# KaranSankla/Lidar_Object_Detection

Hardware: AMD Instinct MI355X
Metric: LiDAR points/sec projected+instance-labelled (higher is better)
Workload: dtype f64

## Files before the change

### lidar_object_detection_amd/csrc/lpf_kernels.hip.h

```cpp
#pragma once
#include <hip/hip_runtime.h>
#include <stdint.h>

#define LPF_BLOCK 256
#define LPF_SEG_QUANTUM 4096
#define LPF_SEG_SMALL 1024
#define LPF_GROUP_SEGS 64
#define LPF_FRM_SHARDS 8
#define LPF_MAX_MASKS_DEV 32
#define LPF_TAB_ROWS 36
#define LPF_TAB_GROUPS 9

struct LpfFrame {
    long long pt_off;
    long long inst_base;
    int N;
    int seg_off;
    int nseg;
    int box_off;
    int B;
    int pad;
    long long cand_off;
    int cand_words;
    int grp_off;
    int shift;
    int pad4;
};

struct LpfParams {
    double T[12];
    double K[9];
    double dmin, dmax;
    int W, H;
    int F, M;
    int seg_pts;
    int nseg_total;
    int nseg_cap;
    int ngrp_cap;
    int oriented;
    long long inst_cap;
    LpfFrame frame0;
    const LpfFrame *frames;
    const LpfFrame *segs;
    const int2 *blks;
    const int4 *cblks;
    int nblk, ncblk;
    int lists_small;
    int csplit;
    const float4 *pts;
    const void *label_img;
    const int4 *rects;
    const uint32_t *rect_grid;
    int rg_cw, rg_cells;
    const double *boxp;
    const float *boxq;
    const unsigned long long *cand;
    int2 *uv;
    uint32_t *label_bits;
    double *depth, *uf, *vf;
    long long *valid_idx;
    int2 *uv_valid;
    uint32_t *label_valid;
    long long *inst_idx;
    int32_t *count_out;
    void *summary;
    unsigned long long *vbal, *mbal;
    uint4 *seg_tab;
    uint4 *grp_tab;
    uint4 *frm_tab;
    uint4 *seg_pre;
    unsigned *cnt;
    float4 *mlist;
    int count_boxes;
    int count_lazy;
    int tile_pts;
};

__device__ __forceinline__ int lpf_lane() { return threadIdx.x & 63; }
__device__ __forceinline__ int lpf_wave() { return threadIdx.x >> 6; }

__device__ __forceinline__ int lpf_xcd_remap(int b, int n)
{
    const int q = n >> 3, r = n & 7, x = b & 7, i = b >> 3;
    return (x < r ? x * (q + 1) : r * (q + 1) + (x - r) * q) + i;
}

__device__ __forceinline__ int lpf_find_frame(const LpfFrame *frames, int F, int sid)
{
    int lo = 0, hi = F;
    while (hi - lo > 1) {
        const int mid = (lo + hi) >> 1;
        if (frames[mid].seg_off <= sid) lo = mid; else hi = mid;
    }
    return lo;
}

__device__ __forceinline__ int lpf_uni(int v) { return __builtin_amdgcn_readfirstlane(v); }
__device__ __forceinline__ long long lpf_uni64(long long v)
{
    return (long long)(((unsigned long long)(unsigned)lpf_uni((int)((unsigned long long)v >> 32)) << 32) | (unsigned)lpf_uni((int)v));
}
__device__ __forceinline__ LpfFrame lpf_frame_record(const LpfFrame &by_value, const LpfFrame *table, const bool many, const int idx)
{
    LpfFrame fr = by_value;
    if (many) {
        const LpfFrame t = table[lpf_uni(idx)];
        fr.pt_off = lpf_uni64(t.pt_off); fr.inst_base = lpf_uni64(t.inst_base); fr.N = lpf_uni(t.N); fr.seg_off = lpf_uni(t.seg_off);
        fr.nseg = lpf_uni(t.nseg); fr.box_off = lpf_uni(t.box_off); fr.B = lpf_uni(t.B); fr.pad = lpf_uni(t.pad);
        fr.cand_off = lpf_uni64(t.cand_off); fr.cand_words = lpf_uni(t.cand_words); fr.grp_off = lpf_uni(t.grp_off); fr.shift = lpf_uni(t.shift);
    }
    return fr;
}

__device__ __forceinline__ int32_t lpf_sat_i32(double r)
{
    int v;
    asm("v_cvt_i32_f64 %0, %1" : "=v"(v) : "v"(r));
    return (r != r) ? INT32_MIN : v;
}

__device__ __forceinline__ unsigned lpf_expo(double x) { return ((unsigned)__double2hiint(x) >> 20) & 0x7ffu; }

__device__ __forceinline__ void lpf_div2(double qx, double qy, double ad, double &uf, double &vf)
{
    const unsigned ea = lpf_expo(ad), ex = lpf_expo(qx), ey = lpf_expo(qy);
    const unsigned lo = min(ea, min(ex, ey)), hi = max(ea, max(ex, ey));
    if (lo >= 723u && hi <= 1323u) {
        double r = __builtin_amdgcn_rcp(ad);
        double e = fma(-ad, r, 1.0); r = fma(r, e, r);
        e = fma(-ad, r, 1.0);        r = fma(r, e, r);
        double q = qx * r; double s = fma(-ad, q, qx); uf = fma(s, r, q);
        q = qy * r;        s = fma(-ad, q, qy);        vf = fma(s, r, q);
    } else {
        uf = qx / ad;
        vf = qy / ad;
    }
}

__device__ __forceinline__ void lpf_project_point(const LpfParams &P, float fx, float fy, float fz,
                                                  double &uf, double &vf, double &d)
{
    const double x = (double)fx, y = (double)fy, z = (double)fz;
    double cx = P.T[0] * x; cx = fma(P.T[1], y, cx); cx = fma(P.T[2],  z, cx); cx = cx + P.T[3];
    double cy = P.T[4] * x; cy = fma(P.T[5], y, cy); cy = fma(P.T[6],  z, cy); cy = cy + P.T[7];
    double cz = P.T[8] * x; cz = fma(P.T[9], y, cz); cz = fma(P.T[10], z, cz); cz = cz + P.T[11];
    double qx = P.K[0] * cx; qx = fma(P.K[1], cy, qx); qx = fma(P.K[2], cz, qx);
    double qy = P.K[3] * cx; qy = fma(P.K[4], cy, qy); qy = fma(P.K[5], cz, qy);
    d = P.K[6] * cx; d = fma(P.K[7], cy, d); d = fma(P.K[8], cz, d);
    if (d == 0.0) d = -1e-6;
    lpf_div2(qx, qy, fabs(d), uf, vf);
}

__device__ __forceinline__ void lpf_project_point_mem(const double *__restrict__ TK, float fx, float fy, float fz,
                                                      double &uf, double &vf, double &d)
{
    const double x = (double)fx, y = (double)fy, z = (double)fz;
    double cx = TK[0] * x; cx = fma(TK[1], y, cx); cx = fma(TK[2],  z, cx); cx = cx + TK[3];
    double cy = TK[4] * x; cy = fma(TK[5], y, cy); cy = fma(TK[6],  z, cy); cy = cy + TK[7];
    double cz = TK[8] * x; cz = fma(TK[9], y, cz); cz = fma(TK[10], z, cz); cz = cz + TK[11];
    double qx = TK[12] * cx; qx = fma(TK[13], cy, qx); qx = fma(TK[14], cz, qx);
    double qy = TK[15] * cx; qy = fma(TK[16], cy, qy); qy = fma(TK[17], cz, qy);
    d = TK[18] * cx; d = fma(TK[19], cy, d); d = fma(TK[20], cz, d);
    if (d == 0.0) d = -1e-6;
    lpf_div2(qx, qy, fabs(d), uf, vf);
}

__device__ __forceinline__ unsigned lpf_f32_to_u8(float v)
{
    int t;
    if (!(v > -2147483904.0f && v < 2147483648.0f)) t = INT32_MIN; else t = (int)v;
    return (unsigned)t & 0xFFu;
}

template <typename T, int MODE>
__device__ __forceinline__ bool lpf_member(T v)
{
    if (MODE == 0) return v != 0;
    if (MODE == 1) return lpf_f32_to_u8((float)v) != 0u;
    if (MODE == 3) return (float)v > 0.5f;
    return lpf_f32_to_u8((float)v * 255.0f) == 255u;
}

template <typename T, int MODE> struct LpfDirect { };
template <typename LT> struct LpfIsDirect { static constexpr bool value = false; };
template <typename T, int MODE> struct LpfIsDirect<LpfDirect<T, MODE> > { static constexpr bool value = true; };

template <typename T, int MODE> struct LpfDirectRect { };
template <typename LT> struct LpfIsDirectRect { static constexpr bool value = false; };
template <typename T, int MODE> struct LpfIsDirectRect<LpfDirectRect<T, MODE> > { static constexpr bool value = true; };
template <typename T, int MODE> struct LpfIsDirect<LpfDirectRect<T, MODE> > { static constexpr bool value = true; };

template <typename LT>
struct LpfLabelSrc {
    typedef LT elem;
    static __device__ __forceinline__ uint32_t get(const elem *__restrict__ img, const LpfParams &, const int pix, const int4 *, int, int) { return (uint32_t)img[pix]; }
    static __device__ __forceinline__ size_t frame_stride(const LpfParams &P) { return (size_t)P.W * (size_t)P.H; }
};
template <typename T, int MODE>
struct LpfLabelSrc<LpfDirect<T, MODE> > {
    typedef T elem;
    static __device__ __forceinline__ uint32_t get(const elem *__restrict__ msk, const LpfParams &P, const int pix, const int4 *__restrict__ rc,
                                                   const int ui, const int vi)
    {
        const size_t hw = (size_t)P.W * (size_t)P.H;
        uint32_t l = 0;
        for (int m0 = 0; m0 < P.M; m0 += 8) {
            T v[8];
#pragma unroll
            for (int j = 0; j < 8; ++j) v[j] = msk[(size_t)min(m0 + j, P.M - 1) * hw + pix];
#pragma unroll
            for (int j = 0; j < 8; ++j)
                if (m0 + j < P.M && lpf_member<T, MODE>(v[j])) l |= 1u << (m0 + j);
        }
        if (rc && l) {
            uint32_t rest = l;
            while (rest) {
                const int m = __ffs(rest) - 1;
                rest &= rest - 1u;
                const int4 q = rc[m];
                if (!(ui >= q.x && ui < q.z && vi >= q.y && vi < q.w)) l &= ~(1u << m);
            }
        }
        return l;
    }
    static __device__ __forceinline__ size_t frame_stride(const LpfParams &P) { return (size_t)P.M * (size_t)P.W * (size_t)P.H; }
};

template <typename T, int MODE>
struct LpfLabelSrc<LpfDirectRect<T, MODE> > {
    typedef T elem;
    static constexpr int mode = MODE;
    static __device__ __forceinline__ uint32_t get(const elem *__restrict__, const LpfParams &, const int, const int4 *, int, int) { return 0u; }
    static __device__ __forceinline__ size_t frame_stride(const LpfParams &P) { return (size_t)P.M * (size_t)P.W * (size_t)P.H; }
};

#define LPF_F_X4 1u
#define LPF_F_NTLOAD 2u
#define LPF_F_NTSTORE 4u
#define LPF_F_LAB_NOMATH 8u
#define LPF_F_LAB_NOGATHER 16u
#define LPF_F_LAB_NOSTORE 32u

#define LPF_F_LAB_NOBAL 64u
#define LPF_F_LAB_NOTAB 128u

#define LPF_RG_SHIFT 4
#define LPF_RG_CELL (1 << LPF_RG_SHIFT)
__device__ __forceinline__ unsigned lpf_wave_or(unsigned x);

template <int ROWS, unsigned FL, typename LT, bool PRELOADED>
__device__ __forceinline__ void lpf_k1_tile(const LpfParams &P, const int blk, unsigned *s_cnt, float4 (&p)[ROWS])
{
    constexpr int TILE = LPF_BLOCK * ROWS;
    static_assert(LPF_SEG_QUANTUM % TILE == 0 && (LPF_SEG_SMALL % TILE == 0 || ROWS >= 8), "tiles must divide segments (8-row and larger tiles: large geometry only)");
    const int tid = threadIdx.x, lane = lpf_lane(), wave = lpf_wave();
    const int tiles_per_seg = P.seg_pts / TILE;
    const int lb = lpf_xcd_remap(blk, P.nseg_total * tiles_per_seg);
    const int sid = lb / tiles_per_seg;
    LpfFrame fr = P.frame0;
    if (P.F > 1) fr = P.segs[__builtin_amdgcn_readfirstlane(sid)];
    const int f = fr.pad;
    const int sh = fr.shift;
    const long long pbase = fr.pt_off - sh;
    const int seg_start = (sid - fr.seg_off) * P.seg_pts;
    const int seg_end = min(seg_start + P.seg_pts, fr.N + sh);
    const int c = seg_start + (lb - sid * tiles_per_seg) * TILE;
    if (c >= seg_end) return;
    const float4 *__restrict__ pts = P.pts + pbase;
    typedef LpfLabelSrc<LT> Src;
    const typename Src::elem *__restrict__ limg =
        (P.label_img && P.M > 0) ? static_cast<const typename Src::elem *>(P.label_img) + (size_t)f * Src::frame_stride(P) : nullptr;
    const int rows_per_seg = P.seg_pts >> 6;
    if (tid < LPF_TAB_ROWS) s_cnt[tid] = 0;
    __syncthreads();
    unsigned nvalid_w = 0, nmask_w = 0;

    {
        const int wbase = c + wave * (ROWS * 64) + lane;
#pragma unroll
        for (int r = 0; r < ROWS; ++r) {
            if constexpr (PRELOADED) continue;
            const float4 *src = pts + min(wbase + r * 64, seg_end - 1);
            if (FL & LPF_F_NTLOAD) {
                typedef float f4v __attribute__((ext_vector_type(4)));
                const f4v t = __builtin_nontemporal_load(reinterpret_cast<const f4v *>(src));
                p[r] = make_float4(t.x, t.y, t.z, t.w);
            } else {
                p[r] = *src;
            }
        }
        uint32_t lab[ROWS];
        bool valid[ROWS];
        constexpr bool RECT = LpfIsDirectRect<LT>::value;
        const int4 *__restrict__ rc_f = ((RECT || LpfIsDirect<LT>::value) && P.rects) ? P.rects + (size_t)f * P.M : nullptr;
        const uint32_t *__restrict__ rgrid = (RECT && limg && P.rect_grid) ? P.rect_grid + (size_t)f * P.rg_cells : nullptr;
        const size_t mhw = (size_t)P.W * (size_t)P.H;
        unsigned long long myv = 0, mym = 0;
        auto consume = [&](const int r, uint32_t l, const bool okr) {
            const int idx = wbase + r * 64;
            if (idx >= sh && idx < seg_end && P.label_bits && !(FL & LPF_F_LAB_NOSTORE)) {
                if (FL & LPF_F_NTSTORE) __builtin_nontemporal_store(l, P.label_bits + pbase + idx);
                else P.label_bits[pbase + idx] = l;
            }
            const unsigned long long vb = __ballot(okr);
            const unsigned long long mb = __ballot(l != 0);
            if (lane == r) { myv = vb; mym = mb; }
            if (l && P.mlist && !(FL & LPF_F_LAB_NOSTORE))
                P.mlist[pbase + (wbase - lane) + ((wbase - lane) == 0 ? sh : 0) + nmask_w + __popcll(mb & ((1ull << lane) - 1ull))] =
                    make_float4(p[r].x, p[r].y, p[r].z, __uint_as_float(l));
            nvalid_w += __popcll(vb);
            nmask_w += __popcll(mb);
            while (l) {
                const int m = __ffs(l) - 1;
                l &= l - 1;
                atomicAdd(&s_cnt[2 + m], 1u);
            }
        };
#pragma unroll
        for (int r = 0; r < ROWS; ++r) {
            const int idx = wbase + r * 64;
            const bool live = idx >= sh && idx < seg_end;
            if (FL & LPF_F_X4) asm volatile("" ::"v"(p[r].w));
            double uf, vf, d, ru, rv;
            if (FL & LPF_F_LAB_NOMATH) {
                uf = (double)p[r].x; vf = (double)p[r].y; d = (double)p[r].z;
                ru = uf + 700.0; rv = vf + 100.0;
            } else {
                lpf_project_point(P, p[r].x, p[r].y, p[r].z, uf, vf, d);
                ru = rint(uf); rv = rint(vf);
            }
            const int ui = lpf_sat_i32(ru), vi = lpf_sat_i32(rv);
            const bool ok = live && ((unsigned)ui < (unsigned)P.W) && ((unsigned)vi < (unsigned)P.H) &&
                            (d > P.dmin) && (d < P.dmax);
            valid[r] = ok;
            lab[r] = 0;
            if constexpr (RECT) {
                if (ok && rgrid) lab[r] = rgrid[(vi >> LPF_RG_SHIFT) * P.rg_cw + (ui >> LPF_RG_SHIFT)];
            } else
            if (!(FL & LPF_F_LAB_NOGATHER)) {
                if (ok && limg) lab[r] = Src::get(limg, P, vi * P.W + ui, rc_f, ui, vi);
            }
            if (live && !(FL & LPF_F_LAB_NOSTORE)) {
                const long long g = pbase + idx;
                if (P.uv) {
                    if (FL & LPF_F_NTSTORE) {
                        typedef int i2v __attribute__((ext_vector_type(2)));
                        i2v t; t.x = ui; t.y = vi;
                        __builtin_nontemporal_store(t, reinterpret_cast<i2v *>(P.uv + g));
                    } else {
                        P.uv[g] = make_int2(ui, vi);
                    }
                }
                if (P.depth) P.depth[g] = d;
                if (P.uf) P.uf[g] = uf;
                if (P.vf) P.vf[g] = vf;
            }
        }
#pragma unroll
        for (int r = 0; r < ROWS; ++r) {
            uint32_t l = lab[r];
            if constexpr (RECT) {
                if (__any(l != 0u)) {
                    double uf, vf, d;
                    lpf_project_point(P, p[r].x, p[r].y, p[r].z, uf, vf, d);
                    const int ui = lpf_sat_i32(rint(uf)), vi = lpf_sat_i32(rint(vf));
                    const unsigned pix = (unsigned)(vi * P.W + ui);
                    uint32_t any = lpf_wave_or(l), l2 = 0u;
                    while (any) {
                        const int m = __ffs(any) - 1;
                        any &= any - 1u;
                        const int4 q = rc_f[m];
                        const bool in = ((l >> m) & 1u) && ui >= q.x && ui < q.z && vi >= q.y && vi < q.w;
                        if (__any(in)) {
                            const typename Src::elem *__restrict__ mk = limg + (size_t)m * mhw;
                            if (in && lpf_member<typename Src::elem, Src::mode>(mk[pix])) l2 |= 1u << m;
                        }
                    }
                    l = l2;
                }
            }
            consume(r, l, valid[r]);
        }
        if (lane < ROWS && !(FL & LPF_F_LAB_NOBAL)) {
            const size_t row = (size_t)sid * rows_per_seg + ((c - seg_start) >> 6) + wave * ROWS + lane;
            P.vbal[row] = myv;
            P.mbal[row] = mym;
        }
    }
    if (lane == 0) { atomicAdd(&s_cnt[0], nvalid_w); atomicAdd(&s_cnt[1], nmask_w); }
    __syncthreads();
    if (!(FL & LPF_F_LAB_NOTAB)) {
        if (tid < (2 + P.M + 1) >> 1) {
            const unsigned long long v = (unsigned long long)s_cnt[2 * tid] | ((unsigned long long)s_cnt[2 * tid + 1] << 32);
            if (v) {
                int seg_off = P.frame0.seg_off, grp_off = P.frame0.grp_off, fid = P.frame0.pad;
                if (P.F > 1) { const LpfFrame *e = P.segs + lpf_uni(sid); seg_off = e->seg_off; grp_off = e->grp_off; fid = e->pad; }
                const int k = sid - seg_off, g = tid >> 1, h = tid & 1;
                atomicAdd(reinterpret_cast<unsigned long long *>(P.seg_tab + (size_t)g * P.nseg_cap + sid) + h, v);
                atomicAdd(reinterpret_cast<unsigned long long *>(P.grp_tab + (size_t)g * P.ngrp_cap + grp_off + (k >> 6)) + h, v);
                atomicAdd(reinterpret_cast<unsigned long long *>(P.frm_tab + ((size_t)fid * LPF_FRM_SHARDS + (k & (LPF_FRM_SHARDS - 1))) * LPF_TAB_GROUPS + g) + h, v);
            }
        }
    }
}

template <int ROWS, unsigned FL, typename LT>
__device__ __forceinline__ void lpf_k1_tile(const LpfParams &P, const int blk, unsigned *s_cnt)
{
    float4 p[ROWS];
    lpf_k1_tile<ROWS, FL, LT, false>(P, blk, s_cnt, p);
}

template <int ROWS, unsigned FL, typename LT = uint32_t>
__global__ __launch_bounds__(LPF_BLOCK) void lpf_k1_project_t(const LpfParams P)
{
    __shared__ unsigned s_cnt[LPF_TAB_ROWS];
    lpf_k1_tile<ROWS, FL, LT>(P, (int)blockIdx.x, s_cnt);
}

#define LPF_K1_FLAGS (LPF_F_X4 | LPF_F_NTLOAD | LPF_F_NTSTORE)

__device__ __forceinline__ bool lpf_oriented_inside(double px, double py, double pz, const double *__restrict__ b)
{
    const double rx = px - b[0], ry = py - b[1], rz = pz - b[2];
    const bool exact_ok = b[15] != 0.0;
#pragma unroll
    for (int a = 0; a < 3; ++a) {
        const double v0 = b[3 + 4 * a], v1 = b[4 + 4 * a], v2 = b[5 + 4 * a], vv = b[6 + 4 * a];
        double d = v1 * ry; d = fma(v0, rx, d); d = fma(v2, rz, d);
        bool in;
        if (exact_ok && !(fabs(d) < 1e-200 && d != 0.0)) {
            in = (d >= 0.0) && (d <= vv);
        } else {
            const double t = d / vv;
            in = (t >= 0.0) && (t <= 1.0);
        }
        if (!in) return false;
    }
    return true;
}

__device__ __forceinline__ bool lpf_aabb_inside(double px, double py, double pz, const double *__restrict__ b)
{
    return (px >= b[0]) && (px <= b[3]) && (py >= b[1]) && (py <= b[4]) && (pz >= b[2]) && (pz <= b[5]);
}

__device__ __forceinline__ unsigned lpf_rl(unsigned v, int l) { return (unsigned)__builtin_amdgcn_readlane((int)v, l); }
__device__ __forceinline__ float lpf_rlf(float v, int l) { return __int_as_float(__builtin_amdgcn_readlane(__float_as_int(v), l)); }
__device__ __forceinline__ unsigned long long lpf_rl64(unsigned long long v, int l)
{
    return (unsigned long long)lpf_rl((unsigned)v, l) | ((unsigned long long)lpf_rl((unsigned)(v >> 32), l) << 32);
}
#define LPF_DPP_ADD(x, ctrl, rows) ((x) + (unsigned)__builtin_amdgcn_update_dpp(0, (int)(x), (ctrl), (rows), 0xf, false))
__device__ __forceinline__ unsigned lpf_wave_sum(unsigned x)
{
    x = LPF_DPP_ADD(x, 0xB1, 0xf);
    x = LPF_DPP_ADD(x, 0x4E, 0xf);
    x = LPF_DPP_ADD(x, 0x141, 0xf);
    x = LPF_DPP_ADD(x, 0x140, 0xf);
    x = LPF_DPP_ADD(x, 0x142, 0xa);
    x = LPF_DPP_ADD(x, 0x143, 0xc);
    return lpf_rl(x, 63);
}
__device__ __forceinline__ unsigned lpf_sum8(unsigned x)
{
    x = LPF_DPP_ADD(x, 0xB1, 0xf);
    x = LPF_DPP_ADD(x, 0x4E, 0xf);
    x = LPF_DPP_ADD(x, 0x141, 0xf);
    return lpf_rl(x, 0);
}
__device__ __forceinline__ unsigned lpf_wave_or(unsigned x)
{
#define LPF_DPP_OR(x, ctrl, rows) ((x) | (unsigned)__builtin_amdgcn_update_dpp(0, (int)(x), (ctrl), (rows), 0xf, false))
    x = LPF_DPP_OR(x, 0xB1, 0xf); x = LPF_DPP_OR(x, 0x4E, 0xf); x = LPF_DPP_OR(x, 0x141, 0xf); x = LPF_DPP_OR(x, 0x140, 0xf);
    x = LPF_DPP_OR(x, 0x142, 0xa); x = LPF_DPP_OR(x, 0x143, 0xc);
#undef LPF_DPP_OR
    return lpf_rl(x, 63);
}

__device__ __forceinline__ void lpf_block_excl4(const unsigned sum[4], unsigned excl[4], unsigned all[4],
                                                unsigned (*s_wsum)[4], int lane, int wave)
{
    unsigned inc[4];
#pragma unroll
    for (int j = 0; j < 4; ++j) {
        unsigned x = sum[j];
#pragma unroll
        for (int o = 1; o < 64; o <<= 1) {
            const unsigned t = __shfl_up(x, o);
            if (lane >= o) x += t;
        }
        inc[j] = x;
        if (lane == 63) s_wsum[wave][j] = x;
    }
    __syncthreads();
#pragma unroll
    for (int j = 0; j < 4; ++j) {
        unsigned wo = 0, a = 0;
#pragma unroll
        for (int w = 0; w < 4; ++w) { const unsigned t = s_wsum[w][j]; if (w < wave) wo += t; a += t; }
        excl[j] = wo + inc[j] - sum[j];
        all[j] = a;
    }
    __syncthreads();
}

__global__ __launch_bounds__(LPF_BLOCK) void lpf_scan_segments(const LpfParams P)
{
    __shared__ unsigned s_toff[LPF_TAB_GROUPS][LPF_BLOCK][4];
    __shared__ unsigned s_wsum[4][4], s_tot[LPF_TAB_ROWS], s_off[LPF_TAB_ROWS];
    const int f = blockIdx.x, tid = threadIdx.x, lane = lpf_lane(), wave = lpf_wave();
    const LpfFrame fr = lpf_frame_record(P.frame0, P.frames, P.F > 1, f);
    const int seg_lo = fr.seg_off, seg_hi = fr.seg_off + fr.nseg;
    const int ngroups = (2 + P.M + 3) >> 2;
    const int R = (fr.nseg + LPF_BLOCK - 1) / LPF_BLOCK;
    const int my_lo = min(seg_lo + tid * R, seg_hi), my_hi = min(my_lo + R, seg_hi);
    for (int g = 0; g < ngroups; ++g) {
        const uint4 *__restrict__ row = P.seg_tab + (size_t)g * P.nseg_cap;
        unsigned sum[4] = {0, 0, 0, 0};
#pragma unroll 8
        for (int sg = my_lo; sg < my_hi; ++sg) {
            const uint4 v = row[sg];
            sum[0] += v.x; sum[1] += v.y; sum[2] += v.z; sum[3] += v.w;
        }
        unsigned excl[4], all[4];
        lpf_block_excl4(sum, excl, all, s_wsum, lane, wave);
#pragma unroll
        for (int j = 0; j < 4; ++j) { s_toff[g][tid][j] = excl[j]; if (tid == 0) s_tot[4 * g + j] = all[j]; }
    }
    __syncthreads();
    if (tid < LPF_TAB_ROWS) {
        const bool used = tid < 4 * ngroups;
        unsigned off = 0;
        if (used) for (int c = 2; c < tid; ++c) off += s_tot[c];
        s_off[tid] = off;
    }
    __syncthreads();
    for (int g = 0; g < ngroups; ++g) {
        const uint4 *__restrict__ row = P.seg_tab + (size_t)g * P.nseg_cap;
        uint4 *__restrict__ pre = P.seg_pre + (size_t)g * P.nseg_cap;
        unsigned run[4];
#pragma unroll
        for (int j = 0; j < 4; ++j) run[j] = s_off[4 * g + j] + s_toff[g][tid][j];
#pragma unroll 8
        for (int sg = my_lo; sg < my_hi; ++sg) {
            const uint4 v = row[sg];
            pre[sg] = make_uint4(run[0], run[1], run[2], run[3]);
            run[0] += v.x; run[1] += v.y; run[2] += v.z; run[3] += v.w;
        }
    }
}

#define LPF_LISTS_WAVES 4
#define LPF_LIST_CAP 1024


__device__ __forceinline__ void lpf_bits_to_list(unsigned long long rowbits, unsigned rowbase, int lane, unsigned short *lst)
{
    unsigned pos = rowbase;
    const unsigned short tag = (unsigned short)(lane * 64);
    while (rowbits) {
        const int b = __ffsll((long long)rowbits) - 1;
        rowbits &= rowbits - 1ull;
        lst[pos++] = (unsigned short)(tag + b);
    }
}

template <bool PRE, int STEP>
__device__ __forceinline__ void lpf_list_prefix(const LpfParams &P, const LpfFrame &fr, const int sid, unsigned &bef, unsigned &tot)
{
    const int lane = lpf_lane();
    const int ngroups = (2 + P.M + 3) >> 2;
    const int k = sid - fr.seg_off;
    bef = 0; tot = 0;
    if (PRE) {
        uint4 q = make_uint4(0u, 0u, 0u, 0u);
        if (lane < ngroups) q = P.seg_pre[(size_t)lane * P.nseg_cap + sid];
        const int g = min(lane >> 2, LPF_TAB_GROUPS - 1);
        const unsigned x = __shfl(q.x, g), y = __shfl(q.y, g), z = __shfl(q.z, g), w = __shfl(q.w, g);
        bef = ((lane & 3) == 0) ? x : ((lane & 3) == 1) ? y : ((lane & 3) == 2) ? z : w;
    } else {
        const int gi = k >> 6, j = k & 63;
        for (int g0 = 0; g0 < ngroups; g0 += STEP) {
            uint4 a[STEP], b[STEP], t[STEP];
#pragma unroll
            for (int u = 0; u < STEP; ++u) {
                const int g = g0 + u;
                a[u] = make_uint4(0u, 0u, 0u, 0u); b[u] = a[u]; t[u] = a[u];
                if (g < ngroups) {
                    if (lane < j) a[u] = P.seg_tab[(size_t)g * P.nseg_cap + fr.seg_off + (gi << 6) + lane];
                    if (lane < gi) b[u] = P.grp_tab[(size_t)g * P.ngrp_cap + fr.grp_off + lane];
                    if (lane < LPF_FRM_SHARDS) t[u] = P.frm_tab[((size_t)fr.pad * LPF_FRM_SHARDS + lane) * LPF_TAB_GROUPS + g];
                }
            }
#pragma unroll
            for (int u = 0; u < STEP; ++u) {
                const int g = g0 + u;
                if (g >= ngroups) break;
                const unsigned px = lpf_wave_sum(a[u].x + b[u].x), py = lpf_wave_sum(a[u].y + b[u].y), pz = lpf_wave_sum(a[u].z + b[u].z), pw = lpf_wave_sum(a[u].w + b[u].w);
                const unsigned tx = lpf_sum8(t[u].x), ty = lpf_sum8(t[u].y), tz = lpf_sum8(t[u].z), tw = lpf_sum8(t[u].w);
                if ((lane >> 2) == g) {
                    bef = ((lane & 3) == 0) ? px : ((lane & 3) == 1) ? py : ((lane & 3) == 2) ? pz : pw;
                    tot = ((lane & 3) == 0) ? tx : ((lane & 3) == 1) ? ty : ((lane & 3) == 2) ? tz : tw;
                }
            }
        }
    }
}

template <bool PRE>
__device__ __forceinline__ unsigned lpf_list_posreg(const LpfParams &P, const unsigned bef, const unsigned tot)
{
    const int lane = lpf_lane();
    if (PRE) return (unsigned)__shfl((int)bef, (lane + 2) & 63);
    unsigned off = (lane >= 2 && lane < 2 + P.M) ? tot : 0u;
    const unsigned own = off;
#pragma unroll
    for (int o = 1; o < 64; o <<= 1) {
        const unsigned u = __shfl_up(off, o);
        if (lane >= o) off += u;
    }
    return (unsigned)__shfl((int)(off - own + bef), (lane + 2) & 63);
}

template <bool PRE, int STEP>
__device__ __forceinline__ void lpf_lists_wave(const LpfParams &P, const LpfFrame &fr, const int sid, unsigned short *lst)
{
    const int lane = lpf_lane();
    const unsigned long long lt = (1ull << lane) - 1ull;
    const int rps = P.seg_pts >> 6;
    const int k = sid - fr.seg_off;
    unsigned long long vb = 0, mb = 0;
    if (lane < rps) {
        vb = P.vbal[(size_t)sid * rps + lane];
        mb = P.mbal[(size_t)sid * rps + lane];
    }
    unsigned bef, tot;
    lpf_list_prefix<PRE, STEP>(P, fr, sid, bef, tot);
    const int sh = fr.shift;
    const int seg_start = k * P.seg_pts;
    const int seg_end = min(seg_start + P.seg_pts, fr.N + sh);
    const int nrows = (seg_end - seg_start + 63) >> 6;
    if (lane >= nrows) { vb = 0; mb = 0; }
    const unsigned cv = __popcll(vb), cm = __popcll(mb);
    unsigned iv = cv, im = cm;
#pragma unroll
    for (int o = 1; o < 64; o <<= 1) {
        const unsigned tv = __shfl_up(iv, o), tm = __shfl_up(im, o);
        if (lane >= o) { iv += tv; im += tm; }
    }
    const unsigned vbase = iv - cv, mbase = im - cm;
    const unsigned nv = lpf_rl(iv, 63), L = lpf_rl(im, 63);
    const long long run_v = (long long)lpf_rl(bef, 0);

    if (P.valid_idx && nv) {
        long long *__restrict__ dst = P.valid_idx + fr.pt_off + run_v;
        const long long o = fr.pt_off + run_v, g0 = fr.pt_off - sh + seg_start;
        const long long room = (long long)fr.N - run_v;
        if (nv > (unsigned)LPF_LIST_CAP || nv > 6u * (unsigned)nrows) {
            for (int r = 0; r < nrows; ++r) {
                const unsigned long long rv = lpf_rl64(vb, r);
                if (rv == 0ull) continue;
                const long long pos = lpf_rl(vbase, r) + __popcll(rv & lt);
                if (((rv >> lane) & 1ull) && pos < room) {
                    dst[pos] = (long long)(seg_start + r * 64 + lane - sh);
                    if (P.uv_valid) P.uv_valid[o + pos] = P.uv[g0 + r * 64 + lane];
                    if (P.label_valid) P.label_valid[o + pos] = P.label_bits[g0 + r * 64 + lane];
                }
            }
        } else {
            lpf_bits_to_list(vb, vbase, lane, lst);
            __builtin_amdgcn_wave_barrier();
            for (unsigned e = lane; e < nv && (long long)e < room; e += 64) {
                const int pt = seg_start + (int)lst[e] - sh;
                dst[e] = (long long)pt;
                if (P.uv_valid) P.uv_valid[o + e] = P.uv[fr.pt_off + pt];
                if (P.label_valid) P.label_valid[o + e] = P.label_bits[fr.pt_off + pt];
            }
            __builtin_amdgcn_wave_barrier();
        }
    }
    if (L == 0 || P.inst_idx == nullptr) return;

    unsigned posreg = lpf_list_posreg<PRE>(P, bef, tot);
    const float4 *__restrict__ mseg = P.mlist + (fr.pt_off - sh) + seg_start;
    const int rows_per_wave = P.tile_pts >> 8;
    const int rpw_shift = (rows_per_wave == 8) ? 3 : (rows_per_wave == 4) ? 2 : (rows_per_wave == 2) ? 1 : 0;
    const int dead0 = (seg_start == 0) ? sh : 0;

    for (int r0 = 0; r0 < nrows;) {
// ... 1360 lines not shown
```

Measured before the change: 171.8 billion.

## Add fast path for full tiles and batch rect-mask refinement gathers

Adds a specialised FAST path for tiles that lie entirely inside the segment and use only the common outputs (uv plus labels, no depth or float coordinates). That path drops the bounds clamps and per-row liveness checks, turns label gathers into unconditional loads, and ballots validity during projection. For the rect-grid label type it keeps the projected pixel coordinates in registers instead of re-projecting in the refinement loop, and reads rectangles through the scalar constant address space. It also processes mask candidates four at a time so their gathers are issued together. The cost is more code instantiated per template, more register pressure from the extra per-row arrays, and a path split on a runtime condition.

```diff
diff --git a/lidar_object_detection_amd/csrc/lpf_kernels.hip.h b/lidar_object_detection_amd/csrc/lpf_kernels.hip.h
--- a/lidar_object_detection_amd/csrc/lpf_kernels.hip.h
+++ b/lidar_object_detection_amd/csrc/lpf_kernels.hip.h
@@ -247,6 +247,10 @@
 #define LPF_RG_SHIFT 4
 #define LPF_RG_CELL (1 << LPF_RG_SHIFT)
 __device__ __forceinline__ unsigned lpf_wave_or(unsigned x);
+__device__ __forceinline__ unsigned long long lpf_rl64(unsigned long long v, int l);
+template <bool B> struct LpfBool { static constexpr bool value = B; };
+typedef int lpf_int4v __attribute__((ext_vector_type(4)));
+typedef const __attribute__((address_space(4))) lpf_int4v *LpfConstRects;
 
 template <int ROWS, unsigned FL, typename LT, bool PRELOADED>
 __device__ __forceinline__ void lpf_k1_tile(const LpfParams &P, const int blk, unsigned *s_cnt, float4 (&p)[ROWS])
@@ -275,12 +279,21 @@
     __syncthreads();
     unsigned nvalid_w = 0, nmask_w = 0;
 
-    {
+    constexpr bool RECT = LpfIsDirectRect<LT>::value;
+    const int4 *__restrict__ rc_f = ((RECT || LpfIsDirect<LT>::value) && P.rects) ? P.rects + (size_t)(RECT ? lpf_uni(f) : f) * P.M : nullptr;
+    const uint32_t *__restrict__ rgrid = (RECT && limg && P.rect_grid) ? P.rect_grid + (size_t)f * P.rg_cells : nullptr;
+    auto rows = [&](auto fast_tag) {
+        constexpr bool FAST = decltype(fast_tag)::value;
+        constexpr bool STORE = !(FL & LPF_F_LAB_NOSTORE);
+        int2 *const o_uv = P.uv;
+        uint32_t *const o_lab = P.label_bits;
+        double *const o_depth = FAST ? nullptr : P.depth, *const o_uf = FAST ? nullptr : P.uf, *const o_vf = FAST ? nullptr : P.vf;
+        float4 *const o_mlist = P.mlist;
         const int wbase = c + wave * (ROWS * 64) + lane;
 #pragma unroll
         for (int r = 0; r < ROWS; ++r) {
             if constexpr (PRELOADED) continue;
-            const float4 *src = pts + min(wbase + r * 64, seg_end - 1);
+            const float4 *src = pts + (FAST ? wbase + r * 64 : min(wbase + r * 64, seg_end - 1));
             if (FL & LPF_F_NTLOAD) {
                 typedef float f4v __attribute__((ext_vector_type(4)));
                 const f4v t = __builtin_nontemporal_load(reinterpret_cast<const f4v *>(src));
@@ -290,25 +303,35 @@
             }
         }
         uint32_t lab[ROWS];
-        bool valid[ROWS];
-        constexpr bool RECT = LpfIsDirectRect<LT>::value;
-        const int4 *__restrict__ rc_f = ((RECT || LpfIsDirect<LT>::value) && P.rects) ? P.rects + (size_t)f * P.M : nullptr;
-        const uint32_t *__restrict__ rgrid = (RECT && limg && P.rect_grid) ? P.rect_grid + (size_t)f * P.rg_cells : nullptr;
+        bool valid[FAST ? 1 : ROWS];
+        int pu[RECT ? ROWS : 1], pv[RECT ? ROWS : 1];
         const size_t mhw = (size_t)P.W * (size_t)P.H;
         unsigned long long myv = 0, mym = 0;
+        auto store_uv = [&](const long long g, const int ui, const int vi) {
+            if (FL & LPF_F_NTSTORE) {
+                typedef int i2v __attribute__((ext_vector_type(2)));
+                i2v t; t.x = ui; t.y = vi;
+                __builtin_nontemporal_store(t, reinterpret_cast<i2v *>(o_uv + g));
+            } else {
+                o_uv[g] = make_int2(ui, vi);
+            }
+        };
+        auto valid_of = [&](const int r) { return ((lpf_rl64(myv, r) >> lane) & 1ull) != 0ull; };
         auto consume = [&](const int r, uint32_t l, const bool okr) {
             const int idx = wbase + r * 64;
-            if (idx >= sh && idx < seg_end && P.label_bits && !(FL & LPF_F_LAB_NOSTORE)) {
-                if (FL & LPF_F_NTSTORE) __builtin_nontemporal_store(l, P.label_bits + pbase + idx);
-                else P.label_bits[pbase + idx] = l;
-            }
-            const unsigned long long vb = __ballot(okr);
+            if (STORE && (FAST || (idx >= sh && idx < seg_end && o_lab))) {
+                if (FL & LPF_F_NTSTORE) __builtin_nontemporal_store(l, o_lab + pbase + idx);
+                else o_lab[pbase + idx] = l;
+            }
+            unsigned long long vb = 0;
+            if constexpr (!FAST) vb = __ballot(okr);
             const unsigned long long mb = __ballot(l != 0);
-            if (lane == r) { myv = vb; mym = mb; }
-            if (l && P.mlist && !(FL & LPF_F_LAB_NOSTORE))
-                P.mlist[pbase + (wbase - lane) + ((wbase - lane) == 0 ? sh : 0) + nmask_w + __popcll(mb & ((1ull << lane) - 1ull))] =
+            if constexpr (FAST) { if (lane == r) mym = mb; }
+            else if (lane == r) { myv = vb; mym = mb; }
+            if (l && o_mlist && STORE)
+                o_mlist[pbase + (wbase - lane) + ((wbase - lane) == 0 ? sh : 0) + nmask_w + __popcll(mb & ((1ull << lane) - 1ull))] =
                     make_float4(p[r].x, p[r].y, p[r].z, __uint_as_float(l));
-            nvalid_w += __popcll(vb);
+            if constexpr (!FAST) nvalid_w += __popcll(vb);
             nmask_w += __popcll(mb);
             while (l) {
                 const int m = __ffs(l) - 1;
@@ -319,7 +342,7 @@
 #pragma unroll
         for (int r = 0; r < ROWS; ++r) {
             const int idx = wbase + r * 64;
-            const bool live = idx >= sh && idx < seg_end;
+            const bool live = FAST || (idx >= sh && idx < seg_end);
             if (FL & LPF_F_X4) asm volatile("" ::"v"(p[r].w));
             double uf, vf, d, ru, rv;
             if (FL & LPF_F_LAB_NOMATH) {
@@ -332,60 +355,98 @@
             const int ui = lpf_sat_i32(ru), vi = lpf_sat_i32(rv);
             const bool ok = live && ((unsigned)ui < (unsigned)P.W) && ((unsigned)vi < (unsigned)P.H) &&
                             (d > P.dmin) && (d < P.dmax);
-            valid[r] = ok;
+            if constexpr (FAST) {
+                const unsigned long long vb = __ballot(ok);
+                if (lane == r) myv = vb;
+                nvalid_w += __popcll(vb);
+            } else {
+                valid[r] = ok;
+            }
             lab[r] = 0;
             if constexpr (RECT) {
-                if (ok && rgrid) lab[r] = rgrid[(vi >> LPF_RG_SHIFT) * P.rg_cw + (ui >> LPF_RG_SHIFT)];
+                const unsigned cell = ((unsigned)vi >> LPF_RG_SHIFT) * (unsigned)P.rg_cw + ((unsigned)ui >> LPF_RG_SHIFT);
+                if constexpr (FAST) lab[r] = rgrid[ok ? cell : 0u];
+                else if (ok && rgrid) lab[r] = rgrid[cell];
+                pu[r] = ui; pv[r] = vi;
             } else
             if (!(FL & LPF_F_LAB_NOGATHER)) {
-                if (ok && limg) lab[r] = Src::get(limg, P, vi * P.W + ui, rc_f, ui, vi);
-            }
-            if (live && !(FL & LPF_F_LAB_NOSTORE)) {
+                if constexpr (FAST) lab[r] = Src::get(limg, P, ok ? vi * P.W + ui : 0, rc_f, ui, vi);
+                else if (ok && limg) lab[r] = Src::get(limg, P, vi * P.W + ui, rc_f, ui, vi);
+            }
+            if (live && STORE) {
                 const long long g = pbase + idx;
-                if (P.uv) {
-                    if (FL & LPF_F_NTSTORE) {
-                        typedef int i2v __attribute__((ext_vector_type(2)));
-                        i2v t; t.x = ui; t.y = vi;
-                        __builtin_nontemporal_store(t, reinterpret_cast<i2v *>(P.uv + g));
-                    } else {
-                        P.uv[g] = make_int2(ui, vi);
-                    }
+                if constexpr (!RECT) {
+                    if (FAST || o_uv) store_uv(g, ui, vi);
                 }
-                if (P.depth) P.depth[g] = d;
-                if (P.uf) P.uf[g] = uf;
-                if (P.vf) P.vf[g] = vf;
-            }
-        }
-#pragma unroll
-        for (int r = 0; r < ROWS; ++r) {
-            uint32_t l = lab[r];
-            if constexpr (RECT) {
+                if constexpr (!FAST) {
+                    if (o_depth) o_depth[g] = d;
+                    if (o_uf) o_uf[g] = uf;
+                    if (o_vf) o_vf[g] = vf;
+                }
+            }
+        }
+        if constexpr (RECT) {
+#pragma unroll
+            for (int r = 0; r < ROWS; ++r) {
+                uint32_t l = (FAST && !valid_of(r)) ? 0u : lab[r];
                 if (__any(l != 0u)) {
-                    double uf, vf, d;
-                    lpf_project_point(P, p[r].x, p[r].y, p[r].z, uf, vf, d);
-                    const int ui = lpf_sat_i32(rint(uf)), vi = lpf_sat_i32(rint(vf));
-                    const unsigned pix = (unsigned)(vi * P.W + ui);
+                    const LpfConstRects rc_c = reinterpret_cast<LpfConstRects>(reinterpret_cast<uintptr_t>(rc_f));
+                    const int ui = pu[r], vi = pv[r];
+                    const unsigned pix = (unsigned)vi * (unsigned)P.W + (unsigned)ui;
                     uint32_t any = lpf_wave_or(l), l2 = 0u;
                     while (any) {
-                        const int m = __ffs(any) - 1;
-                        any &= any - 1u;
-                        const int4 q = rc_f[m];
-                        const bool in = ((l >> m) & 1u) && ui >= q.x && ui < q.z && vi >= q.y && vi < q.w;
-                        if (__any(in)) {
-                            const typename Src::elem *__restrict__ mk = limg + (size_t)m * mhw;
-                            if (in && lpf_member<typename Src::elem, Src::mode>(mk[pix])) l2 |= 1u << m;
+                        constexpr int NB = 4;
+                        int m[NB];
+                        bool in[NB], some = false;
+#pragma unroll
+                        for (int j = 0; j < NB; ++j) {
+                            const bool has = any != 0u;
+                            m[j] = has ? __ffs(any) - 1 : 0;
+                            any &= any - 1u;
+                            const lpf_int4v q = rc_c[lpf_uni(m[j])];
+                            in[j] = has && ((l >> m[j]) & 1u) && ui >= q.x && ui < q.z && vi >= q.y && vi < q.w;
+                            some = some || in[j];
+                        }
+                        if (__any(some)) {
+                            typename Src::elem v[NB];
+#pragma unroll
+                            for (int j = 0; j < NB; ++j) v[j] = (limg + (size_t)m[j] * mhw)[in[j] ? pix : 0u];
+#pragma unroll
+                            for (int j = 0; j < NB; ++j)
+                                if (in[j] && lpf_member<typename Src::elem, Src::mode>(v[j])) l2 |= 1u << m[j];
                         }
                     }
                     l = l2;
                 }
-            }
-            consume(r, l, valid[r]);
+                lab[r] = l;
+            }
+#pragma unroll
+            for (int r = 0; r < ROWS; ++r) {
+                const int idx = wbase + r * 64;
+                const bool live = FAST || (idx >= sh && idx < seg_end);
+                if (live && STORE) {
+                    const long long g = pbase + idx;
+                    if (FAST || o_uv) store_uv(g, pu[r], pv[r]);
+                }
+                consume(r, lab[r], FAST ? false : valid[r]);
+            }
+        } else {
+#pragma unroll
+            for (int r = 0; r < ROWS; ++r) consume(r, (FAST && !valid_of(r)) ? 0u : lab[r], FAST ? false : valid[r]);
         }
         if (lane < ROWS && !(FL & LPF_F_LAB_NOBAL)) {
             const size_t row = (size_t)sid * rows_per_seg + ((c - seg_start) >> 6) + wave * ROWS + lane;
             P.vbal[row] = myv;
             P.mbal[row] = mym;
         }
+    };
+    const bool full = c >= sh && c + TILE <= seg_end;
+    const bool common = P.uv && P.label_bits && !P.depth && !P.uf && !P.vf && (RECT ? rgrid != nullptr : (limg != nullptr || (FL & LPF_F_LAB_NOGATHER)));
+    if constexpr (PRELOADED || (LpfIsDirect<LT>::value && !RECT)) {
+        rows(LpfBool<false>());
+    } else {
+        if (full && common) rows(LpfBool<true>());
+        else rows(LpfBool<false>());
     }
     if (lane == 0) { atomicAdd(&s_cnt[0], nvalid_w); atomicAdd(&s_cnt[1], nmask_w); }
     __syncthreads();
```

Result: faster. 175.4 billion, median of 6 (+2.1%).
